# facebookresearch/robust_cvd

Measured on AMD Instinct MI355X. Metric: GN/LM iterations/sec (and ms/iter) on 300-frame 384x224 video, 1/2/4/8 GPU, higher is better.
Workload: dtype f64

## Files before the change

include/cvd_hip_debug.h:

```cpp
#ifndef CVD_HIP_DEBUG_H
#define CVD_HIP_DEBUG_H

#include "cvd_hip.h"

#ifdef __cplusplus
extern "C" {
#endif

typedef struct cvd_debug_options {
  uint64_t struct_size;
  int32_t force_iterations;
  int32_t force_sharded_path;
  int32_t pcg_lockstep;
  int32_t stall_fused_tail_once;
} cvd_debug_options;
void cvd_debug_options_default(cvd_debug_options* o);
int32_t cvd_set_debug_options(cvd_handle* h, const cvd_debug_options* o);

int32_t cvd_set_generic_kernels(cvd_handle* h, int32_t enabled);

int32_t cvd_comm_init_local_group(cvd_handle* h, int32_t rank, int32_t world, uint64_t group_key);
int32_t cvd_comm_init_phantom(cvd_handle* h, int32_t rank, int32_t world);

int32_t cvd_block_inverse_debug(cvd_handle* h, int32_t num_blocks, int32_t block_size, const double* a, int32_t variant,
                                float* inverse, int32_t* failed);

int32_t cvd_epipolar_debug(cvd_handle* h, int32_t num_pairs, const int64_t* offsets, const float* loc, double pixel_scale,
                           double threshold_px, int32_t iterations, uint64_t seed, uint8_t* is_static_out,
                           double* fundamental_out, int32_t* best_out, int32_t* counts_out, double* hypotheses_out);
// ... 15 lines not shown
```

robust_cvd_amd/api.py:

```python
import ctypes as C
import os
import sys

from . import build as _build
from .binding import Binding
from .ctypes_types import OptParams, SolveSummary, XformDesc

_lib = None
_variant = None


class SolverOptions(C.Structure):
    _fields_ = [
        ("struct_size", C.c_uint64),
        ("pcg_relative_tolerance", C.c_double),
        ("pcg_max_iterations", C.c_int32),
        ("verbose", C.c_int32),
        ("coarse_level", C.c_int32),
        ("robust_loss", C.c_int32),
        ("dense_matrix_free", C.c_int32),
        ("block_inverse_variant", C.c_int32),
        ("coarse_dense_max_unknowns", C.c_int32),
        ("coarse_rebuild_excess", C.c_int32),
        ("coarse_update_budget", C.c_int64),
# ... 9 lines not shown
        ("temporal_grid_y", C.c_int32),
        ("coarse_temporal_step", C.c_int32),
        ("coarse_over_budget", C.c_int32),
        ("coarse_temporal_min_frames", C.c_int32),
        ("temporal_weight", C.c_double),
    ]


class DebugOptions(C.Structure):
    _fields_ = [
        ("struct_size", C.c_uint64),
        ("force_iterations", C.c_int32),
        ("force_sharded_path", C.c_int32),
        ("pcg_lockstep", C.c_int32),
        ("stall_fused_tail_once", C.c_int32),
    ]


class ConsistencyDesc(C.Structure):
    _fields_ = [
        ("struct_size", C.c_uint64),
        ("precision", C.c_int32),
        ("num_frames", C.c_int32),
        ("num_pairs", C.c_int32),
        ("height", C.c_int32),
        ("width", C.c_int32),
        ("distance_type", C.c_int32),
        ("have_warp", C.c_int32),
        ("reserved", C.c_int32),
        ("lambda_reprojection", C.c_double),
# ... 982 lines not shown
            return None
        n = dims[0]
        a = np.zeros((n, n))
        ai = np.zeros((n, n))
        lam = np.zeros(self.num_frames * self.block_size())
        fl = C.c_int32(0)
        dp = lambda x: x.ctypes.data_as(C.POINTER(C.c_double))
        self._check(self._fn("temporal_debug")(self._h, dims, dp(a), dp(ai), dp(lam), C.byref(fl)))
        return {"NT": n, "S": dims[1], "nn": dims[2], "step": dims[3], "Sx": dims[4], "Sy": dims[5], "a_t": a, "a_t_inverse": ai,
                "lam": lam, "failed": fl.value}

    def path_info(self):
        out = (C.c_int32 * 8)()
        self._check(self._fn("path_info")(self._h, out))
        form = {-1: "none", 0: "exact sparse factor", 1: "exact dense inverse", 2: "temporal pose level"}[out[1]]
        return {"pose_graph_level": form, "depth_grid_level": bool(out[2]), "fused_tail": bool(out[3]), "tail_disabled": bool(out[4]),
                "taps": out[5], "work_items": out[6], "cross_blocks": bool(out[7])}

    def product_launch_debug(self):
        out = (C.c_int32 * 6)()
        self._check(self._fn("product_launch_debug")(self._h, out))
        kind = {-1: "none", 0: "generic list", 1: "fast list", 2: "fast dense", 3: "cross blocks"}[out[3]]
        return {"threads": out[0], "spec": out[1], "kd": out[2], "kind": out[3], "kind_name": kind, "work_items": out[4],
                "num_cu": out[5]}

    def assembly_launch_debug(self):
        import numpy as np
        out = (C.c_int32 * 6)()
        cost = np.zeros(self.num_frames, dtype=np.float64)
        self._check(self._fn("assembly_launch_debug")(self._h, out, cost.ctypes.data_as(C.POINTER(C.c_double))))
        kind = {-1: "none", 0: "generic", 1: "fast list", 2: "fast dense", 3: "dense fold"}[out[3]]
# ... 16 lines not shown
```

robust_cvd_amd/csrc/cvd_api.hip:

```cpp
#include "cvd_host.h"
#include "cvd_coarse.h"

namespace cvd {

static void poseOptimizationStep(cvd_handle* h, const cvd_opt_params& p, double depthDeformReg) {
  solve(h, p, depthDeformReg, PK_POSE_STEP);
  paramsToPoses(h, p);
}

static void poseOptimization(cvd_handle* h, const cvd_opt_params& p) {
  posesToParams(h);
  h->records.clear();
  int ctfRows = p.ctf_long, ctfCols = p.ctf_short;
  int dsoRows = p.dso_long, dsoCols = p.dso_short;
  if (h->aspect >= 1.f) {
    std::swap(ctfCols, ctfRows);
    std::swap(dsoCols, dsoRows);
  }
  int initGrid[3] = {1, 1, 1};
  if (h->ddesc.depth_type == CVD_DEPTH_GRID)
    for (int i = 0; i < 3; ++i) initGrid[i] = h->ddesc.grid_size[i];
  const int Nval = (h->ddesc.depth_type == CVD_DEPTH_IDENTITY) ? 0 : valueNumParams(h->ddesc.value_xform);
  size_t nDmax = static_cast<size_t>(h->nD());
  if (p.coarse_to_fine && h->ddesc.depth_type != CVD_DEPTH_IDENTITY && p.num_steps > 1)
// ... 239 lines not shown
    if (o->coarse_update_budget != h->opt.coarse_update_budget || o->coarse_dense_max_unknowns != h->opt.coarse_dense_max_unknowns ||
        (o->coarse_level == 3) != (h->opt.coarse_level == 3) || o->coarse_temporal_step != h->opt.coarse_temporal_step ||
        o->coarse_over_budget != h->opt.coarse_over_budget || o->coarse_temporal_min_frames != h->opt.coarse_temporal_min_frames ||
        o->pcg_fused_tail != h->opt.pcg_fused_tail)
      h->tableValid = false;
    if (o->constraint_order != h->opt.constraint_order) h->orderGx = h->orderGy = -1;
    h->opt = *o;
  });
}
void cvd_debug_options_default(cvd_debug_options* o) {
  o->struct_size = CVD_STRUCT_STAMP(cvd_debug_options);
  o->force_iterations = 0;
  o->force_sharded_path = 0;
  o->pcg_lockstep = 0;
  o->stall_fused_tail_once = 0;
}
int32_t cvd_set_debug_options(cvd_handle* h, const cvd_debug_options* o) {
  CVD_TRY(h, {
    if (o->struct_size != CVD_STRUCT_STAMP(cvd_debug_options))
      throw std::runtime_error("cvd_debug_options: struct_size does not match this library's cvd_hip_debug.h (start from cvd_debug_options_default)");
    h->dbg = *o;
    h->distForced = h->world == 1 && (h->comm != nullptr || h->localGroup || h->phantom) && o->force_sharded_path != 0;
  });
}
void cvd_comm_unique_id(uint8_t* out128) {
  ncclUniqueId id;
  std::memset(&id, 0, sizeof(id));
  (void)ncclGetUniqueId(&id);
  std::memcpy(out128, &id, sizeof(id));
}
// ... 655 lines not shown
      if (a_t) T.A.download(a_t, n2, s);
      if (a_t_inverse) T.Ainv.download(a_t_inverse, n2, s);
      if (lam) h->dLam.download(lam, static_cast<size_t>(h->F) * h->Bsz(), s);
      int fl = 0;
      T.fail.download(&fl, 1, s);
      HIP_CHECK(hipStreamSynchronize(s));
      if (failed) *failed = fl;
    }
  });
}
int32_t cvd_path_info(cvd_handle* h, int32_t* out8) {
  CVD_TRY(h, {
    out8[0] = h->coarseOn ? 1 : 0;
    out8[1] = !h->coarseOn ? -1 : (h->coarse.temporalPose ? 2 : (h->coarse.denseMode ? 1 : 0));
    out8[2] = h->temporal.on ? 1 : 0;
    out8[3] = h->lastFusedTail ? 1 : 0;
    out8[4] = h->tailDisabled ? 1 : 0;
    out8[5] = h->lastKD;
    out8[6] = static_cast<int32_t>(h->itemFa.size());
    out8[7] = h->lastCross ? 1 : 0;
  });
}
int32_t cvd_product_launch_debug(cvd_handle* h, int32_t* out6) {
  CVD_TRY(h, {
    for (int i = 0; i < 6; ++i) out6[i] = h->lastProduct[i];
  });
}
int32_t cvd_assembly_launch_debug(cvd_handle* h, int32_t* out6, double* cost_frame) {
  CVD_TRY(h, {
    for (int i = 0; i < 6; ++i) out6[i] = h->lastAssembly[i];
    const size_t F = static_cast<size_t>(h->F);
// ... 84 lines not shown
```

robust_cvd_amd/csrc/cvd_host.h:

```cpp
#pragma once

#include <hip/hip_runtime.h>
#include <hip/hip_ext.h>
#include <rccl/rccl.h>
#include <rocblas/rocblas.h>
#include <rocsolver/rocsolver.h>

#include <algorithm>
#include <array>
#include <atomic>
#include <chrono>
#include <condition_variable>
#include <cmath>
#include <cstdarg>
#include <cstdint>
#include <cstdio>
#include <cstdlib>
#include <cstring>
#include <functional>
#include <limits>
#include <map>
#include <memory>
#include <mutex>
#include <set>
// ... 310 lines not shown
  DevBuf<unsigned char> dRegCnt;
  RegCache regCache{};
  DevBuf<FrameConst> dFc;
  DevBuf<int> dFail;
  DevBuf<unsigned long long> dCount;
  double* hScal = nullptr;
  double* hStage[2] = {nullptr, nullptr};
  size_t hStageN[2] = {0, 0};
  double* hPcg = nullptr;
  hipEvent_t pcgEvent[2] = {nullptr, nullptr};

  cvd_solve_summary summary{};
  std::vector<cvd_iteration_record> records;

  bool lastFusedTail = false, lastCross = false;
  int lastKD = 0;
  int lastProduct[6] = {0, 0, 0, -1, 0, 0};
  int lastAssembly[6] = {0, 0, 0, -1, 0, 0};
  bool tailDisabled = false;
  bool forceGeneric = false;

  int timing = 0;
  int timingStride = 1;
  long long timingCounter = 0;
  long long timingCounterKc[16] = {0};
  std::vector<std::pair<hipEvent_t, hipEvent_t>> evPool;
  std::vector<int> evClass;
  std::vector<int> evIter;
  int curPcgIter = -1;
  size_t evUsed = 0;
// ... 348 lines not shown
```

robust_cvd_amd/csrc/cvd_matvec.hip:

```cpp
#include "cvd_host.h"
#include "cvd_pcg.h"
#include "cvd_cross.h"
#include "cvd_triplets.h"

namespace cvd {

bool coarseFusedConsumers() {
  return false;
}
bool fusedExchange(cvd_handle* h, bool withCoarse) { return !withCoarse || h->coarse.denseMode; }
size_t exchangeOffsetQc(const Ctx& c) { return c.h->dist() ? static_cast<size_t>(c.h->framesPadded()) * c.L.B : c.n; }
size_t exchangeOffsetPq(const Ctx& c, bool withDenseCoarse) {
  return exchangeOffsetQc(c) + (withDenseCoarse ? static_cast<size_t>(c.L.F) * kCB : 0);
}
size_t exchangeTemporalCount(cvd_handle* h, bool withCoarse) {
  const TlStep ts = temporalStep(h);
  return (ts.Ainv != nullptr && h->dist() && fusedExchange(h, withCoarse)) ? static_cast<size_t>(h->F) * ts.S : 0;
}
bool ownerShardedUpdate(cvd_handle* h, bool withCoarse) {
  return h->dist() && fusedExchange(h, withCoarse) && h->opt.dist_owner_update != 0;
}
CoarseView coarseView(cvd_handle* h, bool on, bool walk) {
  auto& C = h->coarse;
  CoarseView v = on ? CoarseView{C.pos.p, C.wPtr.p, C.wRow.p, walk ? C.Wb.p : nullptr, C.y.p, C.modeActive.p, C.fail.p, C.c.p}
// ... 176 lines not shown
      const int ct = h->tBegin(KC_COMM_PRODUCT);
      commAllReduce(h, q, c.n, CT_F64, s);
      h->tEnd(ct);
      hipLaunchKernelGGL(k_dot_pq, dim3(c.L.F), dim3(256), 0, s, c.L, pNew, q, h->dScal.p, h->dCounters.p, h->dFdot.p,
                         withCoarse ? h->coarse.qc.p : nullptr, h->coarse.modeActive.p, cc,
                         ts.Ainv != nullptr ? temporalStepDev(h) : static_cast<const TlStep*>(nullptr));
      HIP_CHECK(hipGetLastError());
    }
    h->tEnd(slot);
  }
}

bool pcgTailScope(Ctx& c, bool coarse, int nThreads, size_t& lds, int& ldsFinish, int& ldsScratch) {
  cvd_handle* h = c.h;
  const int F = c.L.F, B = c.L.B;
  if (!h->opt.pcg_fused_tail || h->tailDisabled || h->dist() || B > 256 || h->forceGeneric) return false;
  if (coarse && !h->coarse.denseMode) return false;
  const int split = denseRowSplit(h);
  const TlStep ts = temporalStep(h);
  if (ts.Ainv != nullptr && (ts.S * ts.width > cgUpdatePartDoubles(B, nThreads) || tlRowsLds(ts.NT) > B + cgUpdatePartDoubles(B, nThreads)))
    return false;
  const bool poseT = coarse && h->coarse.temporalPose;
  if (poseT && tlRowsLds(h->coarse.ptN) > B + cgUpdatePartDoubles(B, nThreads)) return false;
  const int grid = F + (coarse && !poseT && split > 0 ? (F + kDenseFramesPerGroup - 1) / kDenseFramesPerGroup : 0) +
                   (ts.Ainv != nullptr ? ts.S * ts.parts : 0) + (poseT ? kCB * tlParts(h->coarse.ptNn) : 0);
  const int update = B + cgUpdatePartDoubles(B, nThreads) + 48 + 17 * kCB;
  const int finish = 3 * B + 8 + kCB + (nThreads / 256 - 1) * 256 + kTlMaxS;
  const int denseEnd = (coarse && !poseT) ? F * kCB + nThreads + 16 : 0;
  ldsFinish = update;
  ldsScratch = std::max(update + finish + (coarse && split < kCB ? denseEnd : 0), denseEnd);
  lds = static_cast<size_t>(ldsScratch + 24) * sizeof(double);
  if (lds > kMaxLds) return false;
  static std::map<std::tuple<int, int, int, size_t>, int> perCuCache;
  static std::mutex cacheMutex;
  int perCu = 0;
  {
    std::lock_guard<std::mutex> lock(cacheMutex);
    const auto key = std::make_tuple(h->device, c.KD, nThreads, lds);
    auto it = perCuCache.find(key);
    if (it == perCuCache.end()) {
      CVD_DISPATCH_KD(c.KD, {
        allowLds((k_pcg_tail<KD>), lds);
        HIP_CHECK(hipOccupancyMaxActiveBlocksPerMultiprocessor(&perCu, reinterpret_cast<const void*>(&k_pcg_tail<KD>), nThreads, lds));
      });
      perCuCache[key] = perCu;
    } else {
      perCu = it->second;
    }
  }
  return static_cast<long long>(perCu) * h->numCU >= grid;
}

void launchPcgTail(Ctx& c, const double* x, const double* pOld, double* pNew, int useBeta, const double* lam, double* q,
                   bool withCoarse, int nThreads, size_t lds, int ldsFinish, int ldsScratch, double tol2) {
  cvd_handle* h = c.h;
  hipStream_t s = h->stream;
  const int F = c.L.F;
  const CoarseView cF = coarseView(h, withCoarse, false);
  const int split = denseRowSplit(h);
  const int finishDoubles = 3 * static_cast<int>(c.L.B) + 8 + kCB + (nThreads / 256 - 1) * 256 + kTlMaxS;
  const TlStep ts = temporalStep(h);
  const bool poseT = withCoarse && h->coarse.temporalPose;
  const DenseStep ds = (withCoarse && !poseT) ? DenseStep{h->coarse.denseInv.p, h->coarse.qc.p, h->coarse.rc.p, h->coarse.c.p, h->coarse.dotPart.p,
                                               h->coarse.modeActive.p, h->coarse.fail.p, split, ldsFinish + finishDoubles,
                                               h->coarse.dotPart.p + F}
                                  : DenseStep{nullptr, nullptr, nullptr, nullptr, nullptr, nullptr, nullptr, kCB, 0, nullptr};
  double* fd = h->dFdot.p;
  const TailUpdate U{h->dMinv.p, h->dDx.p, h->dR.p, h->dZ.p, fd + F, fd + 2 * F, tol2, h->coarse.modeActive.p, h->hPcg,
                     h->dCounters.p + 1, h->dTailBar.p, h->dFdot.p + 4 * static_cast<size_t>(F) + 32, ldsFinish, ldsScratch, ds,
                     ts.Ainv != nullptr ? temporalStepDev(h) : static_cast<const TlStep*>(nullptr),
                     poseT ? poseTemporalStepDev(h) : static_cast<const TlStep*>(nullptr),
                     (c.cross && h->xDiagRows) ? 1 : 0};
  const int grid = F + (withCoarse && !poseT && split > 0 ? (F + kDenseFramesPerGroup - 1) / kDenseFramesPerGroup : 0) +
                   (ts.Ainv != nullptr ? ts.S * ts.parts : 0) + (poseT ? kCB * tlParts(h->coarse.ptNn) : 0);
  const int slot = h->tBegin(KC_CG_UPDATE);
  {
    std::unique_ptr<PersistentGate> gate;
    std::unique_lock<std::mutex> alone(PersistentGate::slot(h->device).m);
    if (liveHandles(h->device) > 1) {
      alone.unlock();
      gate.reset(new PersistentGate(h->device, s));
    }
    CVD_DISPATCH_KD(c.KD, {
      hipLaunchKernelGGL((k_pcg_tail<KD>), dim3(grid), dim3(nThreads), lds, s, c.L, x, h->dMask.p, lam, h->dMedian.p, h->dRegOwner.p,
                         h->dInRange.p, c.cross ? h->dXFiOff.p : h->dFiOff.p, h->dFiList.p, h->dQPart.p, pOld, pNew, h->dScal.p,
                         useBeta, q, fd, c.cross ? static_cast<int>(h->xFa.size()) * 2 : h->qRows, h->regCache, cF,
                         withCoarse ? h->coarse.qc.p : static_cast<double*>(nullptr),
// ... 2 lines not shown
    HIP_CHECK(hipGetLastError());
  }
  h->tEnd(slot);
}

void touchModule_matvec() {
  hipFuncAttributes a;
  (void)hipFuncGetAttributes(&a, reinterpret_cast<const void*>(k_dot_pq));
}

}

#ifdef CVD_TAIL_PROFILE
extern "C" int32_t cvd_debug_tail_profile(unsigned long long* out) {
  (void)hipDeviceSynchronize();
  return hipMemcpyFromSymbol(out, HIP_SYMBOL(cvd::g_tailProf), sizeof(unsigned long long) * 1024 * 8) == hipSuccess ? 0 : 1;
}
#endif
#ifdef CVD_MV_PROFILE
extern "C" int32_t cvd_debug_mv_profile(unsigned long long* out) {
  (void)hipDeviceSynchronize();
  return hipMemcpyFromSymbol(out, HIP_SYMBOL(cvd::g_mvProf), sizeof(unsigned long long) * 4096 * 8) == hipSuccess ? 0 : 1;
}
#endif
```

robust_cvd_amd/csrc/cvd_pcg.h:

```cpp
#pragma once

#include "cvd_kernels.h"

namespace cvd {

inline __global__ void k_lm_diag(Layout L, const double* __restrict__ hdiag, double* __restrict__ scale,
                          int computeScale, double radius, double* __restrict__ lam) {
  const size_t n = static_cast<size_t>(L.F) * L.B;
  const size_t i = static_cast<size_t>(blockIdx.x) * blockDim.x + threadIdx.x;
  if (i >= n) return;
  const double h = hdiag[i];
  if (computeScale) scale[i] = 1.0 / (1.0 + sqrt(h));
  const double s = scale[i];
  if (h == 0.0) {
    lam[i] = 1.0;
  } else {
    const double d = fmin(fmax(s * s * h, 1e-6), 1e32);
    lam[i] = d / (radius * s * s);
  }
}

template <int KD>
inline __global__ __launch_bounds__(256) void k_reg_cache(Layout L, const double* __restrict__ x,
                                                   const float* __restrict__ median,
// ... 39 lines not shown
                                                 const double* __restrict__ Hdiag, double* __restrict__ pqOut,
                                                 int ownFirst, int ownCount, double* __restrict__ sm, TailCarry& carry,
                                                 const TlStep* __restrict__ tsp, double* __restrict__ tlPart) {
  const double sDone = scal[S_DONE];
  const int nT = FUSED ? static_cast<int>(blockDim.x) : 256;
  const int B = L.B;
  double* xf = sm;
  double* pf = xf + B;
  double* qf = pf + B;
  double* red = qf + B;
  double* cl = red + 8;
  const int f = blockIdx.x;
  const int tid = threadIdx.x;
  const double beta = useBeta ? scal[S_BETA] : 0.0;
  const size_t base = static_cast<size_t>(f) * B;
  if (V.Wb != nullptr) {
    if (tid < 64) coarseFrameCorrection(V, f, tid, cl);
  } else if (tid < kCB) {
    cl[tid] = (V.cF != nullptr) ? V.cF[f * kCB + tid] : 0.0;
  }
  constexpr int EPT = FUSED ? 1 : 2;
  double vz[2] = {0.0, 0.0}, vm[2] = {0.0, 0.0}, vp[2] = {0.0, 0.0}, vlam[2] = {0.0, 0.0}, pvReg[2] = {0.0, 0.0};
  const bool tlOn = V.tl != nullptr;
  double* tls = cl + kCB + (FUSED ? ((nT >> 8) - 1) * 256 : 0);
  TlTaps tt[EPT];
  float tlW0 = 0.f;
  int tlV0 = 0, tlEntries = 0;
  if (tlOn) {
    if (tid < V.tlS) tls[tid] = V.tl[static_cast<size_t>(f) * V.tlS + tid];
#pragma unroll
// ... 5 lines not shown
      tlW0 = tsp->elW[tid];
      tlV0 = tsp->elV[tid];
    }
  }
#pragma unroll
  for (int e = 0; e < EPT; ++e) {
    const int i = tid + e * 256;
    if (i < B) {
      vz[e] = z[base + i];
      vm[e] = mask[base + i];
      if (useBeta) vp[e] = pOld[base + i];
      vlam[e] = lam[base + i];
      xf[i] = x[base + i];
    }
  }
  const int e0 = fiOff[f], e1 = fiOff[f + 1];
  double rowSum[2] = {0.0, 0.0};
  double* psum = cl + kCB;
  if (L.includeStatic) {
    if constexpr (FUSED) {
      const int nParts = nT >> 8, part = tid >> 8, i = tid & 255;
      if (i < B && part < nParts) {
        const size_t step = static_cast<size_t>(nParts) * B;
        const double* rowp = qPart + static_cast<size_t>(e0 + part) * B + i;
        double a0 = 0.0, a1 = 0.0, a2 = 0.0, a3 = 0.0;
        int r = e0 + part;
        for (; r + 3 * nParts < e1; r += 4 * nParts, rowp += 4 * step) {
          a0 += rowp[0];
          a1 += rowp[step];
          a2 += rowp[2 * step];
          a3 += rowp[3 * step];
// ... 21 lines not shown
        rowSum[e] = (a0 + a1) + (a2 + a3);
      }
    }
  }
  __syncthreads();
  if (sDone != 0.0) return false;
  if constexpr (FUSED) {
    if (L.includeStatic && tid < B)
      for (int k = 0; k + 1 < (nT >> 8); ++k) rowSum[0] += psum[k * 256 + tid];
  }
#pragma unroll
  for (int e = 0; e < EPT; ++e) {
    const int i = tid + e * 256;
    if (i >= B) continue;
    const double pv = vz[e] + (coarseAtLds(cl, L, i) + (tlOn ? tlAt(tls, tt[e]) : 0.0)) * vm[e] + (useBeta ? beta * vp[e] : 0.0);
    pNew[base + i] = pv;
    pvReg[e] = pv;
    pf[i] = pv * vm[e];
    qf[i] = (L.includeStatic && !(L.intrOpt == kIntrShared && i == 6)) ? rowSum[e] : 0.0;
  }
  __syncthreads();
  if (L.intrOpt == kIntrShared && f == 0 && L.includeStatic) {
    double a = 0.0;
    for (int k = tid; k < nRows; k += nT) a += qPart[static_cast<size_t>(k) * B + 6];
    a = waveSum(a);
    if ((tid & 63) == 0) atomicAdd(&qf[6], a);
    __syncthreads();
  }
  if (Hdiag != nullptr && f >= ownFirst && f < ownFirst + ownCount) {
    const double* Hf = Hdiag + static_cast<size_t>(f) * B * B;
    for (int i = tid; i < B; i += 256) {
      double a0 = 0.0, a1 = 0.0, a2 = 0.0, a3 = 0.0;
      int j = 0;
      for (; j + 3 < B; j += 4) {
        a0 += Hf[static_cast<size_t>(j) * B + i] * pf[j];
        a1 += Hf[static_cast<size_t>(j + 1) * B + i] * pf[j + 1];
        a2 += Hf[static_cast<size_t>(j + 2) * B + i] * pf[j + 2];
        a3 += Hf[static_cast<size_t>(j + 3) * B + i] * pf[j + 3];
      }
      for (; j < B; ++j) a0 += Hf[static_cast<size_t>(j) * B + i] * pf[j];
      qf[i] += (a0 + a1) + (a2 + a3);
    }
    __syncthreads();
  } else if (Hdiag == nullptr && inRange[f]) {
    const int regStride = CVD_DETERMINISTIC ? 64 : nT;
    for (int i = tid; i < rc.nr && tid < regStride; i += regStride) {
      const int n = rc.cnt[static_cast<size_t>(f) * rc.nr + i];
      const size_t e0 = static_cast<size_t>(f) * rc.stride * rc.nr + i;
      double t = 0.0;
      for (int a = 0; a < n; ++a) t += rc.jac[e0 + static_cast<size_t>(a) * rc.nr] * pf[rc.col[e0 + static_cast<size_t>(a) * rc.nr]];
      for (int a = 0; a < n; ++a)
        atomicAdd(&qf[rc.col[e0 + static_cast<size_t>(a) * rc.nr]], rc.jac[e0 + static_cast<size_t>(a) * rc.nr] * t);
    }
  }
  if (L.positionRegSqrt > 0.0 && tid < 3) {
    const double w = L.positionRegSqrt * L.positionRegSqrt;
    const double cf[3] = {1.0, -2.0, 1.0};
    double acc = 0.0;
    for (int o = 0; o < 3; ++o) {
// ... 12 lines not shown
  if (!FUSED && distMode && pqOut == nullptr) {
#pragma unroll
    for (int e = 0; e < EPT; ++e) {
      const int i = tid + e * 256;
      if (i < B) q[base + i] = qf[i] * vm[e] + (distMode == 1 ? vlam[e] * pvReg[e] : 0.0);
    }
    return true;
  }
  double dot = 0.0;
#pragma unroll
  for (int e = 0; e < EPT; ++e) {
    const int i = tid + e * 256;
    if (i >= B) continue;
    const double pv = pvReg[e];
    const double qv = qf[i] * vm[e] + (distMode == 2 ? 0.0 : vlam[e] * pv);
    q[base + i] = qv;
    qf[i] = qv;
    dot += pv * qv;
    if (e == 0) { carry.pv = pv; carry.qv = qv; }
  }
  dot = waveSum(dot);
  if ((tid & 63) == 0 && tid < 256) red[tid >> 6] = dot;
  __syncthreads();
  if (tid == 0) publishPartial(fdot + f, red[0] + red[1] + red[2] + red[3]);
  if (qc != nullptr) {
    coarseRestrict<FUSED>(L, qf, f, tid, V.modeActive, qc);
    if constexpr (!FUSED) {
      __syncthreads();
      coarseColumnProducts(cc, qc + f * kCB, f, tid, 256);
    }
  }
// ... 80 lines not shown
  if (tid == 0) publishPartial(fdot + f, red[0] + red[1] + red[2] + red[3]);
  if (lastBlockArrivesLite(counter, L.F, reinterpret_cast<int*>(red + 6))) {
    const double pq = blockSumPartials(fdot, L.F, red);
    if (tid == 0) {
      scal[S_PQ] = pq;
      scal[S_ALPHA] = scal[S_RZ] / pq;
    }
  }
}

__host__ __device__ inline int cgUpdatePartDoubles(int B, int nThreads) {
  return B > 256 ? nThreads : max(nThreads, 16 * ((B + 3) & ~3));
}

#ifdef CVD_TAIL_PROFILE
__device__ unsigned long long g_tailProf[1024 * 8];
#define TAIL_STAMP(slot) do { if (threadIdx.x == 0) g_tailProf[(blockIdx.x & 1023) * 8 + (slot)] = wall_clock64(); } while (0)
#else
#define TAIL_STAMP(slot) do {} while (0)
#endif

struct NoMid {
  __device__ bool first(double&, double&) { return true; }
  __device__ bool second(double&) { return true; }
  __device__ unsigned int generation() { return 0u; }
};
typedef unsigned int cvd_u32x4 __attribute__((ext_vector_type(4)));
template <bool FUSED, typename Mid>
__device__ __forceinline__ bool tlLevelRows(const TlStep* __restrict__ tsp, int wg, int F, double& alpha, int init, double sDone,
                                            const double* __restrict__ scal, double* __restrict__ sm, Mid& mid) {
  const TlStep ts = *tsp;
  const int tid = threadIdx.x, nThreads = blockDim.x;
  const int wv = tid >> 6, lane = tid & 63, nW = nThreads >> 6;
  const int s = wg / ts.parts, part = wg - s * ts.parts;
  const int aLo = part * ts.span, aHi = min(ts.nn - 1, aLo + ts.span), nA = aHi - aLo + 1;
  const bool ownsLast = part == ts.parts - 1;
  const int par = init ? 1 : (static_cast<int>(scal[S_ITERS]) & 1);
  const double* tin = ts.t + static_cast<size_t>(par) * ts.NT;
  double* tout = ts.t + static_cast<size_t>(par ^ 1) * ts.NT;
  double* qT = sm;
  double* tn = qT + ts.NT;
  double* red = tn + ts.span + 1;
  double rOldPre = 0.0, tOldPre = 0.0;
  if (lane == 0 && !init) {
    const int e = s * ts.nn + aLo + (wv < nA ? wv : 0);
    rOldPre = ts.rT[e];
    tOldPre = tin[e];
  }
  if constexpr (FUSED) {
    if (!mid.second(alpha)) return false;
  }
  const double inv = 1.0 / static_cast<double>(ts.step);
  bool direct = true;
  if constexpr (FUSED) {
    if (ts.rec != nullptr) {
      direct = false;
      const unsigned int gen = mid.generation() + 1u;
      cvd_u32x4* rec = reinterpret_cast<cvd_u32x4*>(ts.rec);
      for (int a = wv; a < ts.nn; a += nW) {
        const int f = (a - 1) * ts.step + 1 + lane;
        const bool in = lane < 2 * ts.step - 1 && f >= 0 && f < F;
        double v = in ? readPartial(ts.sq + static_cast<size_t>(f) * ts.S + s) : 0.0;
        v *= 1.0 - fabs(static_cast<double>(f - a * ts.step)) * inv;
        v = waveSum(in ? v : 0.0);
// ... 41 lines not shown
          const double* src = ts.sq + static_cast<size_t>(min(f + u, fHi)) * ts.S + sp;
          v[u] = FUSED ? readPartial(src) : *src;
        }
#pragma unroll
        for (int u = 0; u < kTlBatch; ++u) {
          const double w = 1.0 - fabs(static_cast<double>(f + u - a * ts.step)) * inv;
          acc[u & 3] += (f + u <= fHi) ? w * v[u] : 0.0;
        }
      }
      qT[sp * ts.nn + a] = (acc[0] + acc[1]) + (acc[2] + acc[3]);
    }
    __syncthreads();
  }
  if (sDone != 0.0) return false;
  if constexpr (FUSED) TAIL_STAMP(5);
  const bool on = *ts.fail == 0;
  for (int k = wv; k < nA; k += nW) {
    const int a = aLo + k, e = s * ts.nn + a;
    const double* row = ts.Ainv + static_cast<size_t>(e) * ts.ld;
    const bool owned = ownsLast || a < aHi;
    double rOld = rOldPre, tOld = tOldPre;
    double acc0 = 0.0, acc1 = 0.0;
    int c = lane;
    if (k != wv && lane == 0 && !init) {
      rOld = ts.rT[e];
      tOld = tin[e];
    }
    for (; c + 64 < ts.NT; c += 128) {
      acc0 += row[c] * qT[c];
      acc1 += row[c + 64] * qT[c + 64];
    }
    if (c < ts.NT) acc0 += row[c] * qT[c];
    const double d = ts.weight * waveSum(acc0 + acc1);
    if (lane == 0) {
      const double rn = init ? qT[e] : rOld - alpha * qT[e];
      const double tv = on ? (init ? d : tOld - alpha * d) : 0.0;
      if (owned) {
        ts.rT[e] = rn;
        tout[e] = tv;
      }
      tn[k] = tv;
      red[k] = owned ? tv * rn : 0.0;
    }
  }
  __syncthreads();
  if constexpr (FUSED) TAIL_STAMP(6);
  const int fLo = aLo * ts.step, fHi = ownsLast ? F : min(F, aHi * ts.step);
// ... 395 lines not shown
  if (threadIdx.x != 0 || scal[S_DONE] != 0.0) return;
  double rz = 0.0, rr = 0.0;
  for (int r = 0; r < world; ++r) {
    rz += parts[2 * r];
    rr += parts[2 * r + 1];
  }
  pcgFinishScalars(scal, 0, rz, rr, tol2, hostMirror);
}

constexpr int kTailBarCopies = 16;
constexpr int kTailBarStride = 1024;
__device__ __forceinline__ unsigned int tailGeneration(const unsigned int* bar) {
  if (threadIdx.x != 0) return 0u;
  return *reinterpret_cast<const volatile unsigned int*>(bar + kTailBarStride * (1 + (blockIdx.x & (kTailBarCopies - 1))));
}
__device__ __forceinline__ unsigned int tailArrive(unsigned int* bar) {
  asm volatile("s_waitcnt vmcnt(0)" ::: "memory");
  __syncthreads();
  if (threadIdx.x != 0) return 0u;
  return __hip_atomic_fetch_add(bar, 1u, __ATOMIC_RELAXED, __HIP_MEMORY_SCOPE_AGENT);
}
__device__ __forceinline__ bool tailWait(unsigned int* bar, unsigned int nGroups, unsigned int gen, unsigned int ticket,
                                         const double* __restrict__ parts, int nParts, double* __restrict__ scratch, double& sum) {
  int* role = reinterpret_cast<int*>(scratch + 16);
  if (threadIdx.x == 0) {
    *role = (ticket == nGroups - 1) ? 2 : 1;
    *reinterpret_cast<unsigned int*>(scratch + 17) = gen;
  }
  __syncthreads();
  gen = *reinterpret_cast<unsigned int*>(scratch + 17);
  if (*role == 2) {
    const double v = blockSumPartials(parts, nParts, scratch);
    if (threadIdx.x == 0) __hip_atomic_store(bar, 0u, __ATOMIC_RELAXED, __HIP_MEMORY_SCOPE_AGENT);
    if (threadIdx.x < kTailBarCopies) {
      cvd_u32x4 rec;
      rec.x = gen + 1u;
      rec.y = static_cast<unsigned int>(__double2loint(v));
      rec.z = static_cast<unsigned int>(__double2hiint(v));
      rec.w = gen + 1u;
      *reinterpret_cast<volatile cvd_u32x4*>(bar + kTailBarStride * (1 + threadIdx.x)) = rec;
    }
    sum = v;
    return true;
  }
  if (threadIdx.x == 0) {
    const volatile cvd_u32x4* mine = reinterpret_cast<const volatile cvd_u32x4*>(bar + kTailBarStride * (1 + (blockIdx.x & (kTailBarCopies - 1))));
    int ok = 1;
    unsigned int spins = 0;
    cvd_u32x4 rec;
    for (;;) {
      rec = *mine;
      if (rec.x == gen + 1u && rec.w == gen + 1u) break;
      __builtin_amdgcn_s_sleep(16);
      ++spins;
      if ((spins & 63u) == 0 && __hip_atomic_load(bar + 1, __ATOMIC_RELAXED, __HIP_MEMORY_SCOPE_AGENT) != 0u) { ok = 0; break; }
      if (spins > (1u << 18)) {
        __hip_atomic_store(bar + 1, 1u, __ATOMIC_RELAXED, __HIP_MEMORY_SCOPE_AGENT);
// ... 17 lines not shown
  double* z;
  double* fdotRZ;
  double* fdotRR;
  double tol2;
  const unsigned char* modeActive;
  double* hostMirror;
  unsigned int* counter;
  unsigned int* gridBar;
  double* pqSlot;
  int ldsFinish;
  int ldsScratch;
  DenseStep ds;
  const TlStep* ts;
  const TlStep* tp;
  int diagInProduct;
};

template <int KD>
inline __global__ __launch_bounds__(1024) __attribute__((amdgpu_waves_per_eu(6))) void k_pcg_tail(Layout L, const double* __restrict__ x,
                                                    const double* __restrict__ mask,
                                                    const double* __restrict__ lam, const float* __restrict__ median,
                                                    const unsigned char* __restrict__ inRange,
                                                    const unsigned char* __restrict__ rangeFlags,
                                                    const int* __restrict__ fiOff, const int* __restrict__ fiList,
                                                    const double* __restrict__ qPart, const double* __restrict__ pOld,
                                                    double* __restrict__ pNew, double* __restrict__ scal, int useBeta,
                                                    double* __restrict__ q, double* __restrict__ fdot, int nRows, RegCache rc,
                                                    CoarseView V, double* __restrict__ qc, const double* __restrict__ Hdiag,
                                                    TailUpdate U) {
  extern __shared__ __attribute__((aligned(16))) double sm[];
  const int f = blockIdx.x;
  const CoarseColumns ccOff{nullptr, nullptr, nullptr, nullptr, nullptr};
  const CoarseStep csOff{nullptr, nullptr, nullptr, nullptr, nullptr, nullptr, nullptr, nullptr, nullptr};
  TAIL_STAMP(0);
  const unsigned int barGen = tailGeneration(U.gridBar);
  unsigned int barTicket = 0u;
  auto first = [&](double& pv, double& qv) -> bool {
    if (f < L.F) {
      TailCarry carry{0.0, 0.0};
      if (!matvecFinishBody<KD, true>(L, x, mask, lam, median, inRange, rangeFlags, fiOff, fiList, qPart, U.z, pOld, pNew, scal,
                                      nullptr, useBeta, q, fdot, 0, nRows, rc, V, qc, ccOff, Hdiag, nullptr, 0, U.diagInProduct ? 0 : L.F,
                                      sm + U.ldsFinish, carry, U.ts, sm + L.B))
        return false;
      pv = carry.pv;
      qv = carry.qv;
    } else if (scal[S_DONE] != 0.0) {
      return false;
    }
    TAIL_STAMP(1);
    barTicket = tailArrive(U.gridBar);
    return true;
  };
  auto second = [&](double& alpha) -> bool {
    double pq;
    TAIL_STAMP(2);
    if (!tailWait(U.gridBar, gridDim.x, barGen, barTicket, fdot, L.F, sm + U.ldsScratch, pq)) return false;
    TAIL_STAMP(3);
    alpha = scal[S_RZ] / pq;
    if (blockIdx.x == 0 && threadIdx.x == 0) {
      scal[S_PQ] = pq;
      scal[S_ALPHA] = alpha;
    }
    return true;
  };
  struct Mid {
    decltype(first)& f1;
    decltype(second)& f2;
    double* scratch;
    __device__ bool first(double& pv, double& qv) { return f1(pv, qv); }
    __device__ bool second(double& alpha) { return f2(alpha); }
    __device__ unsigned int generation() { return *reinterpret_cast<unsigned int*>(scratch + 17); }
  } mid{first, second, sm + U.ldsScratch};
  cgUpdateBody<true>(L, 0, nullptr, U.minv, nullptr, nullptr, scal, U.counter, U.dx, U.r, U.z, U.fdotRZ, U.fdotRR, U.tol2, nullptr,
                     U.modeActive, U.hostMirror, csOff, U.ds, nullptr, sm, mid, 0, L.F, nullptr, U.ts, U.tp);
  TAIL_STAMP(4);
}

inline __global__ void k_apply_step(Layout L, int boundDepth0, const double* __restrict__ x, const double* __restrict__ dx,
                             double* __restrict__ xc) {
  const size_t n = static_cast<size_t>(L.F) * L.B;
  const size_t i = static_cast<size_t>(blockIdx.x) * blockDim.x + threadIdx.x;
  if (i >= n) return;
  double v = x[i] + dx[i];
  if (boundDepth0) {
    const int c = static_cast<int>(i % L.B);
    if (c >= 7 && c < 7 + L.nD && ((c - 7) % L.N) == 0) v = fmax(v, 0.0);
  }
// ... 22 lines not shown
```

Baseline: 333.5.

## Stage temporal inverse rows in LDS during fused PCG tail barrier wait

In the fused PCG tail kernel, each temporal-level workgroup now copies its rows of the temporal inverse matrix into LDS before waiting on the grid barrier, then reads them from LDS in the matvec, so the global loads overlap the barrier stall. The barrier is restructured: the last-arriving group reduces the partial dot products in one wave inside tailArrive, and the pNew/q stores are moved after arrival so they leave the critical path. rzOld is read early. Staging needs more LDS, so it is used only when occupancy still keeps the whole grid resident, with a debug switch to disable it.

```diff
diff --git a/include/cvd_hip_debug.h b/include/cvd_hip_debug.h
--- a/include/cvd_hip_debug.h
+++ b/include/cvd_hip_debug.h
@@ -13,6 +13,7 @@
   int32_t force_sharded_path;
   int32_t pcg_lockstep;
   int32_t stall_fused_tail_once;
+  int32_t tail_no_row_staging;
 } cvd_debug_options;
 void cvd_debug_options_default(cvd_debug_options* o);
 int32_t cvd_set_debug_options(cvd_handle* h, const cvd_debug_options* o);
diff --git a/robust_cvd_amd/api.py b/robust_cvd_amd/api.py
--- a/robust_cvd_amd/api.py
+++ b/robust_cvd_amd/api.py
@@ -47,6 +47,7 @@
         ("force_sharded_path", C.c_int32),
         ("pcg_lockstep", C.c_int32),
         ("stall_fused_tail_once", C.c_int32),
+        ("tail_no_row_staging", C.c_int32),
     ]
 
 
@@ -1059,7 +1060,8 @@
         out = (C.c_int32 * 8)()
         self._check(self._fn("path_info")(self._h, out))
         form = {-1: "none", 0: "exact sparse factor", 1: "exact dense inverse", 2: "temporal pose level"}[out[1]]
-        return {"pose_graph_level": form, "depth_grid_level": bool(out[2]), "fused_tail": bool(out[3]), "tail_disabled": bool(out[4]),
+        return {"pose_graph_level": form, "depth_grid_level": bool(out[2]), "fused_tail": bool(out[3] & 1), "tail_rows_staged": bool(out[3] & 2),
+                "tail_disabled": bool(out[4]),
                 "taps": out[5], "work_items": out[6], "cross_blocks": bool(out[7])}
 
     def product_launch_debug(self):
diff --git a/robust_cvd_amd/csrc/cvd_api.hip b/robust_cvd_amd/csrc/cvd_api.hip
--- a/robust_cvd_amd/csrc/cvd_api.hip
+++ b/robust_cvd_amd/csrc/cvd_api.hip
@@ -277,6 +277,7 @@
   o->force_sharded_path = 0;
   o->pcg_lockstep = 0;
   o->stall_fused_tail_once = 0;
+  o->tail_no_row_staging = 0;
 }
 int32_t cvd_set_debug_options(cvd_handle* h, const cvd_debug_options* o) {
   CVD_TRY(h, {
@@ -962,7 +963,7 @@
     out8[0] = h->coarseOn ? 1 : 0;
     out8[1] = !h->coarseOn ? -1 : (h->coarse.temporalPose ? 2 : (h->coarse.denseMode ? 1 : 0));
     out8[2] = h->temporal.on ? 1 : 0;
-    out8[3] = h->lastFusedTail ? 1 : 0;
+    out8[3] = h->lastFusedTail ? (h->tailStageRows ? 3 : 1) : 0;
     out8[4] = h->tailDisabled ? 1 : 0;
     out8[5] = h->lastKD;
     out8[6] = static_cast<int32_t>(h->itemFa.size());
diff --git a/robust_cvd_amd/csrc/cvd_host.h b/robust_cvd_amd/csrc/cvd_host.h
--- a/robust_cvd_amd/csrc/cvd_host.h
+++ b/robust_cvd_amd/csrc/cvd_host.h
@@ -348,6 +348,7 @@
   std::vector<cvd_iteration_record> records;
 
   bool lastFusedTail = false, lastCross = false;
+  bool tailStageRows = false;
   int lastKD = 0;
   int lastProduct[6] = {0, 0, 0, -1, 0, 0};
   int lastAssembly[6] = {0, 0, 0, -1, 0, 0};
diff --git a/robust_cvd_amd/csrc/cvd_matvec.hip b/robust_cvd_amd/csrc/cvd_matvec.hip
--- a/robust_cvd_amd/csrc/cvd_matvec.hip
+++ b/robust_cvd_amd/csrc/cvd_matvec.hip
@@ -214,6 +214,7 @@
 bool pcgTailScope(Ctx& c, bool coarse, int nThreads, size_t& lds, int& ldsFinish, int& ldsScratch) {
   cvd_handle* h = c.h;
   const int F = c.L.F, B = c.L.B;
+  h->tailStageRows = false;
   if (!h->opt.pcg_fused_tail || h->tailDisabled || h->dist() || B > 256 || h->forceGeneric) return false;
   if (coarse && !h->coarse.denseMode) return false;
   const int split = denseRowSplit(h);
@@ -228,27 +229,40 @@
   const int finish = 3 * B + 8 + kCB + (nThreads / 256 - 1) * 256 + kTlMaxS;
   const int denseEnd = (coarse && !poseT) ? F * kCB + nThreads + 16 : 0;
   ldsFinish = update;
-  ldsScratch = std::max(update + finish + (coarse && split < kCB ? denseEnd : 0), denseEnd);
-  lds = static_cast<size_t>(ldsScratch + 24) * sizeof(double);
-  if (lds > kMaxLds) return false;
+  const int unstaged = std::max(update + finish + (coarse && split < kCB ? denseEnd : 0), denseEnd);
+  int stagedEnd = 0;
+  if (ts.Ainv != nullptr) stagedEnd = std::max(stagedEnd, tlStagedLds(ts.NT));
+  if (poseT) stagedEnd = std::max(stagedEnd, tlStagedLds(h->coarse.ptN));
   static std::map<std::tuple<int, int, int, size_t>, int> perCuCache;
   static std::mutex cacheMutex;
-  int perCu = 0;
-  {
+  auto resident = [&](size_t bytes) {
+    if (bytes > kMaxLds) return false;
+    int perCu = 0;
     std::lock_guard<std::mutex> lock(cacheMutex);
-    const auto key = std::make_tuple(h->device, c.KD, nThreads, lds);
+    const auto key = std::make_tuple(h->device, c.KD, nThreads, bytes);
     auto it = perCuCache.find(key);
     if (it == perCuCache.end()) {
       CVD_DISPATCH_KD(c.KD, {
-        allowLds((k_pcg_tail<KD>), lds);
-        HIP_CHECK(hipOccupancyMaxActiveBlocksPerMultiprocessor(&perCu, reinterpret_cast<const void*>(&k_pcg_tail<KD>), nThreads, lds));
+        allowLds((k_pcg_tail<KD>), bytes);
+        HIP_CHECK(hipOccupancyMaxActiveBlocksPerMultiprocessor(&perCu, reinterpret_cast<const void*>(&k_pcg_tail<KD>), nThreads, bytes));
       });
       perCuCache[key] = perCu;
     } else {
       perCu = it->second;
     }
-  }
-  return static_cast<long long>(perCu) * h->numCU >= grid;
+    return static_cast<long long>(perCu) * h->numCU >= grid;
+  };
+  if (stagedEnd > 0 && h->dbg.tail_no_row_staging == 0) {
+    ldsScratch = std::max(unstaged, stagedEnd);
+    lds = static_cast<size_t>(ldsScratch + 24) * sizeof(double);
+    if (resident(lds)) {
+      h->tailStageRows = true;
+      return true;
+    }
+  }
+  ldsScratch = unstaged;
+  lds = static_cast<size_t>(ldsScratch + 24) * sizeof(double);
+  return resident(lds);
 }
 
 void launchPcgTail(Ctx& c, const double* x, const double* pOld, double* pNew, int useBeta, const double* lam, double* q,
@@ -270,7 +284,7 @@
                      h->dCounters.p + 1, h->dTailBar.p, h->dFdot.p + 4 * static_cast<size_t>(F) + 32, ldsFinish, ldsScratch, ds,
                      ts.Ainv != nullptr ? temporalStepDev(h) : static_cast<const TlStep*>(nullptr),
                      poseT ? poseTemporalStepDev(h) : static_cast<const TlStep*>(nullptr),
-                     (c.cross && h->xDiagRows) ? 1 : 0};
+                     (c.cross && h->xDiagRows) ? 1 : 0, h->tailStageRows ? 1 : 0};
   const int grid = F + (withCoarse && !poseT && split > 0 ? (F + kDenseFramesPerGroup - 1) / kDenseFramesPerGroup : 0) +
                    (ts.Ainv != nullptr ? ts.S * ts.parts : 0) + (poseT ? kCB * tlParts(h->coarse.ptNn) : 0);
   const int slot = h->tBegin(KC_CG_UPDATE);
@@ -303,7 +317,7 @@
 #ifdef CVD_TAIL_PROFILE
 extern "C" int32_t cvd_debug_tail_profile(unsigned long long* out) {
   (void)hipDeviceSynchronize();
-  return hipMemcpyFromSymbol(out, HIP_SYMBOL(cvd::g_tailProf), sizeof(unsigned long long) * 1024 * 8) == hipSuccess ? 0 : 1;
+  return hipMemcpyFromSymbol(out, HIP_SYMBOL(cvd::g_tailProf), sizeof(unsigned long long) * 1024 * 16) == hipSuccess ? 0 : 1;
 }
 #endif
 #ifdef CVD_MV_PROFILE
diff --git a/robust_cvd_amd/csrc/cvd_pcg.h b/robust_cvd_amd/csrc/cvd_pcg.h
--- a/robust_cvd_amd/csrc/cvd_pcg.h
+++ b/robust_cvd_amd/csrc/cvd_pcg.h
@@ -77,6 +77,13 @@
   const int tid = threadIdx.x;
   const double beta = useBeta ? scal[S_BETA] : 0.0;
   const size_t base = static_cast<size_t>(f) * B;
+  int e0 = 0, e1 = 0;
+  bool regRowsOn = false;
+  if constexpr (FUSED) {
+    e0 = fiOff[f];
+    e1 = fiOff[f + 1];
+    regRowsOn = Hdiag == nullptr && inRange[f];
+  }
   if (V.Wb != nullptr) {
     if (tid < 64) coarseFrameCorrection(V, f, tid, cl);
   } else if (tid < kCB) {
@@ -112,7 +119,10 @@
       xf[i] = x[base + i];
     }
   }
-  const int e0 = fiOff[f], e1 = fiOff[f + 1];
+  if constexpr (!FUSED) {
+    e0 = fiOff[f];
+    e1 = fiOff[f + 1];
+  }
   double rowSum[2] = {0.0, 0.0};
   double* psum = cl + kCB;
   if (L.includeStatic) {
@@ -164,7 +174,7 @@
     const int i = tid + e * 256;
     if (i >= B) continue;
     const double pv = vz[e] + (coarseAtLds(cl, L, i) + (tlOn ? tlAt(tls, tt[e]) : 0.0)) * vm[e] + (useBeta ? beta * vp[e] : 0.0);
-    pNew[base + i] = pv;
+    if constexpr (!FUSED) pNew[base + i] = pv;
     pvReg[e] = pv;
     pf[i] = pv * vm[e];
     qf[i] = (L.includeStatic && !(L.intrOpt == kIntrShared && i == 6)) ? rowSum[e] : 0.0;
@@ -192,7 +202,7 @@
       qf[i] += (a0 + a1) + (a2 + a3);
     }
     __syncthreads();
-  } else if (Hdiag == nullptr && inRange[f]) {
+  } else if (FUSED ? regRowsOn : (Hdiag == nullptr && inRange[f])) {
     const int regStride = CVD_DETERMINISTIC ? 64 : nT;
     for (int i = tid; i < rc.nr && tid < regStride; i += regStride) {
       const int n = rc.cnt[static_cast<size_t>(f) * rc.nr + i];
@@ -235,7 +245,7 @@
     if (i >= B) continue;
     const double pv = pvReg[e];
     const double qv = qf[i] * vm[e] + (distMode == 2 ? 0.0 : vlam[e] * pv);
-    q[base + i] = qv;
+    if constexpr (!FUSED) q[base + i] = qv;
     qf[i] = qv;
     dot += pv * qv;
     if (e == 0) { carry.pv = pv; carry.qv = qv; }
@@ -346,8 +356,8 @@
 }
 
 #ifdef CVD_TAIL_PROFILE
-__device__ unsigned long long g_tailProf[1024 * 8];
-#define TAIL_STAMP(slot) do { if (threadIdx.x == 0) g_tailProf[(blockIdx.x & 1023) * 8 + (slot)] = wall_clock64(); } while (0)
+__device__ unsigned long long g_tailProf[1024 * 16];
+#define TAIL_STAMP(slot) do { if (threadIdx.x == 0) g_tailProf[(blockIdx.x & 1023) * 16 + (slot)] = wall_clock64(); } while (0)
 #else
 #define TAIL_STAMP(slot) do {} while (0)
 #endif
@@ -356,7 +366,9 @@
   __device__ bool first(double&, double&) { return true; }
   __device__ bool second(double&) { return true; }
   __device__ unsigned int generation() { return 0u; }
+  __device__ bool stageRows() { return false; }
 };
+__host__ __device__ inline int tlStagedLds(int NT) { return tlRowsLds(NT) + (kTlSpan + 1) * NT; }
 typedef unsigned int cvd_u32x4 __attribute__((ext_vector_type(4)));
 template <bool FUSED, typename Mid>
 __device__ __forceinline__ bool tlLevelRows(const TlStep* __restrict__ tsp, int wg, int F, double& alpha, int init, double sDone,
@@ -379,7 +391,35 @@
     rOldPre = ts.rT[e];
     tOldPre = tin[e];
   }
+  double* stage = sm + tlRowsLds(ts.NT);
+  bool staged = false;
   if constexpr (FUSED) {
+    staged = mid.stageRows();
+    if (staged) {
+      constexpr int kStageBatch = 8;
+      for (int k = wv; k < nA; k += nW) {
+        const double* row = ts.Ainv + static_cast<size_t>(s * ts.nn + aLo + k) * ts.ld;
+        double* dst = stage + static_cast<size_t>(k) * ts.NT;
+        for (int c0 = 0; c0 < ts.NT; c0 += 64 * kStageBatch) {
+          double v[kStageBatch];
+#pragma unroll
+          for (int u = 0; u < kStageBatch; ++u) {
+            const int c = c0 + u * 64 + lane;
+            v[u] = row[min(c, ts.NT - 1)];
+          }
+#pragma unroll
+          for (int u = 0; u < kStageBatch; ++u) {
+            const int c = c0 + u * 64 + lane;
+            if (c < ts.NT) dst[c] = v[u];
+          }
+        }
+      }
+    }
+    TAIL_STAMP(8);
+  }
+  bool on = false;
+  if constexpr (FUSED) {
+    on = *ts.fail == 0;
     if (!mid.second(alpha)) return false;
   }
   const double inv = 1.0 / static_cast<double>(ts.step);
@@ -451,7 +491,7 @@
   }
   if (sDone != 0.0) return false;
   if constexpr (FUSED) TAIL_STAMP(5);
-  const bool on = *ts.fail == 0;
+  if constexpr (!FUSED) on = *ts.fail == 0;
   for (int k = wv; k < nA; k += nW) {
     const int a = aLo + k, e = s * ts.nn + a;
     const double* row = ts.Ainv + static_cast<size_t>(e) * ts.ld;
@@ -463,11 +503,20 @@
       rOld = ts.rT[e];
       tOld = tin[e];
     }
-    for (; c + 64 < ts.NT; c += 128) {
-      acc0 += row[c] * qT[c];
-      acc1 += row[c + 64] * qT[c + 64];
-    }
-    if (c < ts.NT) acc0 += row[c] * qT[c];
+    if (staged) {
+      const double* srow = stage + static_cast<size_t>(k) * ts.NT;
+      for (; c + 64 < ts.NT; c += 128) {
+        acc0 += srow[c] * qT[c];
+        acc1 += srow[c + 64] * qT[c + 64];
+      }
+      if (c < ts.NT) acc0 += srow[c] * qT[c];
+    } else {
+      for (; c + 64 < ts.NT; c += 128) {
+        acc0 += row[c] * qT[c];
+        acc1 += row[c + 64] * qT[c + 64];
+      }
+      if (c < ts.NT) acc0 += row[c] * qT[c];
+    }
     const double d = ts.weight * waveSum(acc0 + acc1);
     if (lane == 0) {
       const double rn = init ? qT[e] : rOld - alpha * qT[e];
@@ -893,23 +942,26 @@
   if (threadIdx.x != 0) return 0u;
   return *reinterpret_cast<const volatile unsigned int*>(bar + kTailBarStride * (1 + (blockIdx.x & (kTailBarCopies - 1))));
 }
-__device__ __forceinline__ unsigned int tailArrive(unsigned int* bar) {
+__device__ __forceinline__ void tailArrive(unsigned int* bar, unsigned int nGroups, unsigned int gen, const double* __restrict__ parts,
+                                           int nParts, double* __restrict__ scratch) {
   asm volatile("s_waitcnt vmcnt(0)" ::: "memory");
   __syncthreads();
-  if (threadIdx.x != 0) return 0u;
-  return __hip_atomic_fetch_add(bar, 1u, __ATOMIC_RELAXED, __HIP_MEMORY_SCOPE_AGENT);
-}
-__device__ __forceinline__ bool tailWait(unsigned int* bar, unsigned int nGroups, unsigned int gen, unsigned int ticket,
-                                         const double* __restrict__ parts, int nParts, double* __restrict__ scratch, double& sum) {
-  int* role = reinterpret_cast<int*>(scratch + 16);
-  if (threadIdx.x == 0) {
-    *role = (ticket == nGroups - 1) ? 2 : 1;
-    *reinterpret_cast<unsigned int*>(scratch + 17) = gen;
-  }
-  __syncthreads();
-  gen = *reinterpret_cast<unsigned int*>(scratch + 17);
-  if (*role == 2) {
-    const double v = blockSumPartials(parts, nParts, scratch);
+  if (threadIdx.x >= 64) return;
+  unsigned int ticket = 0u;
+  if (threadIdx.x == 0) ticket = __hip_atomic_fetch_add(bar, 1u, __ATOMIC_RELAXED, __HIP_MEMORY_SCOPE_AGENT);
+  ticket = __builtin_amdgcn_readfirstlane(ticket);
+  gen = __builtin_amdgcn_readfirstlane(gen);
+  const bool last = ticket == nGroups - 1;
+  if (last) {
+    double a = 0.0;
+    for (int k0 = threadIdx.x; k0 < nParts + static_cast<int>(threadIdx.x); k0 += 8 * 64) {
+      double w[8];
+#pragma unroll
+      for (int u = 0; u < 8; ++u) w[u] = k0 + u * 64 < nParts ? readPartial(parts + k0 + u * 64) : 0.0;
+#pragma unroll
+      for (int u = 0; u < 8; ++u) a += w[u];
+    }
+    const double v = waveSum(a);
     if (threadIdx.x == 0) __hip_atomic_store(bar, 0u, __ATOMIC_RELAXED, __HIP_MEMORY_SCOPE_AGENT);
     if (threadIdx.x < kTailBarCopies) {
       cvd_u32x4 rec;
@@ -919,7 +971,19 @@
       rec.w = gen + 1u;
       *reinterpret_cast<volatile cvd_u32x4*>(bar + kTailBarStride * (1 + threadIdx.x)) = rec;
     }
-    sum = v;
+    if (threadIdx.x == 0) scratch[18] = v;
+  }
+  if (threadIdx.x == 0) {
+    *reinterpret_cast<int*>(scratch + 16) = last ? 2 : 1;
+    *reinterpret_cast<unsigned int*>(scratch + 17) = gen;
+  }
+}
+__device__ __forceinline__ bool tailWait(unsigned int* bar, double* __restrict__ scratch, double& sum) {
+  int* role = reinterpret_cast<int*>(scratch + 16);
+  __syncthreads();
+  const unsigned int gen = *reinterpret_cast<unsigned int*>(scratch + 17);
+  if (*role == 2) {
+    sum = scratch[18];
     return true;
   }
   if (threadIdx.x == 0) {
@@ -967,6 +1031,7 @@
   const TlStep* ts;
   const TlStep* tp;
   int diagInProduct;
+  int stageRows;
 };
 
 template <int KD>
@@ -987,7 +1052,7 @@
   const CoarseStep csOff{nullptr, nullptr, nullptr, nullptr, nullptr, nullptr, nullptr, nullptr, nullptr};
   TAIL_STAMP(0);
   const unsigned int barGen = tailGeneration(U.gridBar);
-  unsigned int barTicket = 0u;
+  const double rzOld = scal[S_RZ];
   auto first = [&](double& pv, double& qv) -> bool {
     if (f < L.F) {
       TailCarry carry{0.0, 0.0};
@@ -1001,15 +1066,20 @@
       return false;
     }
     TAIL_STAMP(1);
-    barTicket = tailArrive(U.gridBar);
+    tailArrive(U.gridBar, gridDim.x, barGen, fdot, L.F, sm + U.ldsScratch);
+    TAIL_STAMP(10);
+    if (f < L.F && static_cast<int>(threadIdx.x) < L.B) {
+      pNew[static_cast<size_t>(f) * L.B + threadIdx.x] = pv;
+      q[static_cast<size_t>(f) * L.B + threadIdx.x] = qv;
+    }
     return true;
   };
   auto second = [&](double& alpha) -> bool {
     double pq;
     TAIL_STAMP(2);
-    if (!tailWait(U.gridBar, gridDim.x, barGen, barTicket, fdot, L.F, sm + U.ldsScratch, pq)) return false;
+    if (!tailWait(U.gridBar, sm + U.ldsScratch, pq)) return false;
     TAIL_STAMP(3);
-    alpha = scal[S_RZ] / pq;
+    alpha = rzOld / pq;
     if (blockIdx.x == 0 && threadIdx.x == 0) {
       scal[S_PQ] = pq;
       scal[S_ALPHA] = alpha;
@@ -1023,7 +1093,9 @@
     __device__ bool first(double& pv, double& qv) { return f1(pv, qv); }
     __device__ bool second(double& alpha) { return f2(alpha); }
     __device__ unsigned int generation() { return *reinterpret_cast<unsigned int*>(scratch + 17); }
-  } mid{first, second, sm + U.ldsScratch};
+    bool stage;
+    __device__ bool stageRows() { return stage; }
+  } mid{first, second, sm + U.ldsScratch, U.stageRows != 0};
   cgUpdateBody<true>(L, 0, nullptr, U.minv, nullptr, nullptr, scal, U.counter, U.dx, U.r, U.z, U.fdotRZ, U.fdotRR, U.tol2, nullptr,
                      U.modeActive, U.hostMirror, csOff, U.ds, nullptr, sm, mid, 0, L.F, nullptr, U.ts, U.tp);
   TAIL_STAMP(4);
```

Result: faster. 340.1, median of 6 (+2.0%).
